# chngdickson/ov2slam

Measured on AMD Instinct MI355X. Metric: tracked_frames_per_sec, higher is better.
Workload: dtype u8/s16 fixed-point + f32

## Files before the change

### ov2slam_amd/csrc/klt.hip

```cpp
#include <cstdlib>

#include "ov2_internal.h"
#include "ov2_wave.h"

using namespace ov2wave;

namespace {

struct klt_params {
    int win, nlevels, max_iter;
    int wave_prio;
    double eps2;
    float err_th;
    double fb_th;
    float min_eig_thr;
    int rule33;
};

#define W_BITS 14

__device__ __forceinline__ void lk_weights(float a, float b, int &w00, int &w01, int &w10, int &w11)
{
    w00 = (int)__builtin_rintf((1.f - a) * (1.f - b) * (float)(1 << W_BITS));
    w01 = (int)__builtin_rintf(a * (1.f - b) * (float)(1 << W_BITS));
// ... 38 lines not shown
    constexpr int GSEG = klt_lds<WIN>::GSEG, NS = (WIN + 1) * GSEG, NK = (NS + GL - 1) / GL;
#pragma unroll
    for (int k = 0; k < NK; ++k) {
        const int sg = sub + GL * k;
        if (sg < NS) {
            const int row = sg / GSEG, part = sg - row * GSEG;
            *reinterpret_cast<uint4 *>(lg + sg * 16) =
                ld_b128(reinterpret_cast<const unsigned char *>(src + (size_t)row * gstride) + part * 16);
        }
    }
}

struct lds_col {
    const unsigned *q;
    unsigned sh;
};
__device__ __forceinline__ lds_col lds_col_of(const unsigned char *row0 , int byte_off)
{
    lds_col c;
    c.q = reinterpret_cast<const unsigned *>(row0 + (byte_off & ~3));
    c.sh = (unsigned)byte_off & 3u;
    return c;
}
__device__ __forceinline__ unsigned lds_pair(const lds_col &c, int row)
{
    const unsigned *q = c.q + 4 * row;
    return __builtin_amdgcn_alignbyte(q[1], q[0], c.sh);
}

typedef short ov2_s16x2 __attribute__((ext_vector_type(2)));

__device__ __forceinline__ int dot2(unsigned a, unsigned b, int c)
{
    return __builtin_amdgcn_sdot2(__builtin_bit_cast(ov2_s16x2, a), __builtin_bit_cast(ov2_s16x2, b), c, false);
}
__device__ __forceinline__ int dot2k(unsigned a, unsigned b, int k)
{
    int r;
    asm("v_dot2_i32_i16 %0, %1, %2, %3" : "=v"(r) : "v"(a), "v"(b), "s"(k));
    return r;
}
__device__ __forceinline__ unsigned spread_u8x2(unsigned t) { return __builtin_amdgcn_perm(0u, t, 0x0c010c00u); }
__device__ __forceinline__ unsigned pack_lo16(unsigned a, unsigned b) { return __builtin_amdgcn_perm(b, a, 0x05040100u); }
__device__ __forceinline__ unsigned pack_hi16(unsigned a, unsigned b) { return __builtin_amdgcn_perm(b, a, 0x07060302u); }
__device__ __forceinline__ unsigned pk_sub16(unsigned a, unsigned b)
{
    return __builtin_bit_cast(unsigned, (ov2_s16x2)(__builtin_bit_cast(ov2_s16x2, a) - __builtin_bit_cast(ov2_s16x2, b)));
}

typedef unsigned short ov2_u16x2 __attribute__((ext_vector_type(2)));
__device__ __forceinline__ unsigned pk_add16(unsigned a, unsigned b)
{
    return __builtin_bit_cast(unsigned, (ov2_u16x2)(__builtin_bit_cast(ov2_u16x2, a) + __builtin_bit_cast(ov2_u16x2, b)));
}
__device__ __forceinline__ unsigned pk_mul16(unsigned a, unsigned k)
{
    return __builtin_bit_cast(unsigned, (ov2_u16x2)(__builtin_bit_cast(ov2_u16x2, a) * (ov2_u16x2)((unsigned short)k)));
}
__device__ __forceinline__ unsigned pk_mad16(unsigned a, unsigned k, unsigned c)
{
    return __builtin_bit_cast(unsigned, (ov2_u16x2)(__builtin_bit_cast(ov2_u16x2, a) * (ov2_u16x2)((unsigned short)k) + __builtin_bit_cast(ov2_u16x2, c)));
}

template <int SH>
__device__ __forceinline__ unsigned shr_pack_hi(unsigned keep, unsigned acc)
{
    asm("v_lshrrev_b32_sdwa %0, %2, %1 dst_sel:WORD_1 dst_unused:UNUSED_PRESERVE src0_sel:DWORD src1_sel:DWORD" : "+v"(keep) : "v"(acc), "n"(SH));
    return keep;
}
template <int SH>
__device__ __forceinline__ unsigned ashr_pack_hi(unsigned keep, int acc)
{
    asm("v_ashrrev_i32_sdwa %0, %2, %1 dst_sel:WORD_1 dst_unused:UNUSED_PRESERVE src0_sel:DWORD src1_sel:DWORD" : "+v"(keep) : "v"(acc), "n"(SH));
    return keep;
}

struct level_ptrs {
    const unsigned char *img;
    const int *grad;
    int istride, gstride, w, h, rows;
    const unsigned char *base;
    unsigned img_o, grad_o;
};

__device__ __forceinline__ level_ptrs level_of(const ov2_pyr_view &v, int l, int b)
{
    level_ptrs p;
    const ov2_level_desc &L = v.lv[l];
    p.img = v.base + L.img_off + L.img_bstride * b;
    p.grad = reinterpret_cast<const int *>(v.base + L.grad_off + L.grad_bstride * b);
    p.istride = L.istride; p.gstride = L.gstride; p.w = L.w; p.h = L.h; p.rows = L.rows;
    p.base = v.base; p.img_o = (unsigned)(L.img_off + L.img_bstride * b); p.grad_o = (unsigned)(L.grad_off + L.grad_bstride * b);
    return p;
}

template <int WIN, int GL>
__device__ __forceinline__ int lk_level(const level_ptrs &I, const level_ptrs &J, int pad, int level, int max_level,
                                        bool run, float kx, float ky, float &nx_io, float &ny_io, int &status,
                                        float &err, const klt_params &P, int sub, unsigned &passes,
                                        unsigned char *lwI, unsigned char *lwJ, unsigned char *lg)
{
    constexpr int GROW = klt_lds<WIN>::GSEG * 4;
    constexpr int OC = WIN < GL ? WIN : GL;
    constexpr int NE = (WIN - OC) * WIN;
    constexpr int NR = (NE + GL - 1) / GL;
    constexpr int NRP = (NR + 1) / 2;
    constexpr int NP = (WIN + 1) / 2;
    const float FLT_SCALE = 1.f / (float)(1 << 20);
    const float half = (float)(WIN - 1) * 0.5f;
    const float lscale = __builtin_ldexpf(1.f, -level);
    float px = kx * lscale, py = ky * lscale;
    float nx, ny;
    if (level == max_level) { nx = nx_io * lscale; ny = ny_io * lscale; }
    else { nx = nx_io * 2.f; ny = ny_io * 2.f; }
    if (run) { nx_io = nx; ny_io = ny; }

    px -= half; py -= half;
    const int ipx = (int)floorf(px), ipy = (int)floorf(py);
    if (run && (ipx < -WIN || ipx >= I.w || ipy < -WIN || ipy >= I.h)) {
        if (level == 0) { status = 0; err = 0.f; }
        run = false;
    }
    if (!__any(run)) return 0;
    if (run) passes += 1u;
    int w00, w01, w10, w11;
    lk_weights(px - (float)ipx, py - (float)ipy, w00, w01, w10, w11);

    const bool col = sub < OC;
    const int sc = col ? sub : 0;
    unsigned Iv2[NP], Ix2[NP], Iy2[NP];
    unsigned IvE[NRP > 0 ? NRP : 1], IxE[NRP > 0 ? NRP : 1], IyE[NRP > 0 ? NRP : 1];
    int eoff[NR > 0 ? NR : 1];
    int sA11 = 0, sA12 = 0, sA22 = 0;
    {
        const unsigned W01 = pack_lo16((unsigned)w00, (unsigned)w01), W23 = pack_lo16((unsigned)w10, (unsigned)w11);
        const int bx0 = run ? (OV2_LM + ipx) : OV2_LM, by = run ? (ipy + pad) : pad;
        {
            const float sx = nx - half, sy = ny - half;
            const int inx0 = (int)floorf(sx), iny0 = (int)floorf(sy);
            const bool in0 = run && !(inx0 < -WIN || inx0 >= J.w || iny0 < -WIN || iny0 >= J.h);
            __syncthreads();
            const int jx0 = OV2_LM + (in0 ? inx0 : 0);
            stage_u8<WIN, GL>(I.img + (size_t)by * I.istride + (bx0 & ~3), I.istride, lwI, sub);
            stage_grad<WIN, GL>(I.grad + (size_t)by * I.gstride + bx0, I.gstride, lg, sub);
            stage_u8<WIN, GL>(J.img + (size_t)((in0 ? iny0 : 0) + pad) * J.istride + (jx0 & ~3), J.istride, lwJ, sub);
            __syncthreads();
        }
        const lds_col ci = lds_col_of(lwI, (bx0 & 3) + sc);
        const int *gp = reinterpret_cast<const int *>(lg) + sc;
        unsigned T = spread_u8x2(lds_pair(ci, 0));
        unsigned GX, GY;
        {
            const unsigned g0 = (unsigned)gp[0], g1 = (unsigned)gp[1];
            GX = pack_lo16(g0, g1); GY = pack_hi16(g0, g1);
        }
        const bool on = run && col;
        unsigned piv = 0, pix = 0, piy = 0;
#pragma unroll
        for (int y = 0; y < WIN; ++y) {
            gp += GROW;
            const unsigned B = spread_u8x2(lds_pair(ci, y + 1));
            const unsigned h0 = (unsigned)gp[0], h1 = (unsigned)gp[1];
            const unsigned HX = pack_lo16(h0, h1), HY = pack_hi16(h0, h1);
            const unsigned iv = (unsigned)dot2(B, W23, dot2k(T, W01, 1 << (W_BITS - 5 - 1))) >> (W_BITS - 5);
            int ix = dot2(HX, W23, dot2k(GX, W01, 1 << (W_BITS - 1))) >> W_BITS;
            int iy = dot2(HY, W23, dot2k(GY, W01, 1 << (W_BITS - 1))) >> W_BITS;
            if (y & 1) {
                Iv2[y >> 1] = pack_lo16(piv, iv); Ix2[y >> 1] = pack_lo16(pix, (unsigned)ix); Iy2[y >> 1] = pack_lo16(piy, (unsigned)iy);
            } else if (y == WIN - 1) {
                Iv2[y >> 1] = iv; Ix2[y >> 1] = (unsigned)ix & 0xffffu; Iy2[y >> 1] = (unsigned)iy & 0xffffu;
            } else {
                piv = iv; pix = (unsigned)ix; piy = (unsigned)iy;
            }
            T = B; GX = HX; GY = HY;
        }
        {
            const unsigned onm = on ? 0xffffffffu : 0u;
#pragma unroll
            for (int q = 0; q < NP; ++q) {
                Ix2[q] &= onm; Iy2[q] &= onm;
                sA11 = dot2(Ix2[q], Ix2[q], sA11); sA12 = dot2(Ix2[q], Iy2[q], sA12); sA22 = dot2(Iy2[q], Iy2[q], sA22);
            }
        }
#pragma unroll
        for (int r = 0; r < NR; ++r) {
            const int e = sub + GL * r;
            const bool ev = e < NE;
            const int ec = ev ? e : 0;
            const int ecol = OC + ec / WIN, erow = ec - (ec / WIN) * WIN;
            eoff[r] = erow * 16 + ecol;
            const lds_col ce = lds_col_of(lwI + erow * 16, (bx0 & 3) + ecol);
            const int *gpe = reinterpret_cast<const int *>(lg) + erow * GROW + ecol;
            const unsigned T0 = spread_u8x2(lds_pair(ce, 0)), T1 = spread_u8x2(lds_pair(ce, 1));
            const unsigned g0 = (unsigned)gpe[0], g1 = (unsigned)gpe[1];
            const unsigned h0 = (unsigned)gpe[GROW], h1 = (unsigned)gpe[GROW + 1];
            const unsigned iv = (unsigned)dot2(T1, W23, dot2k(T0, W01, 1 << (W_BITS - 5 - 1))) >> (W_BITS - 5);
            int ix = dot2(pack_lo16(h0, h1), W23, dot2k(pack_lo16(g0, g1), W01, 1 << (W_BITS - 1))) >> W_BITS;
            int iy = dot2(pack_hi16(h0, h1), W23, dot2k(pack_hi16(g0, g1), W01, 1 << (W_BITS - 1))) >> W_BITS;
            if (!(run && ev)) { ix = 0; iy = 0; }
            sA11 += __mul24(ix, ix); sA12 += __mul24(ix, iy); sA22 += __mul24(iy, iy);
            if (r & 1) {
                IvE[r >> 1] = pack_lo16(piv, iv); IxE[r >> 1] = pack_lo16(pix, (unsigned)ix); IyE[r >> 1] = pack_lo16(piy, (unsigned)iy);
            } else if (r == NR - 1) {
                IvE[r >> 1] = iv; IxE[r >> 1] = (unsigned)ix & 0xffffu; IyE[r >> 1] = (unsigned)iy & 0xffffu;
            } else {
                piv = iv; pix = (unsigned)ix; piy = (unsigned)iy;
            }
        }
    }
    const float A11 = (float)(double)row_sum_i32<GL>(sA11) * FLT_SCALE;
    const float A12 = (float)(double)row_sum_i32<GL>(sA12) * FLT_SCALE;
    const float A22 = (float)(double)row_sum_i32<GL>(sA22) * FLT_SCALE;
    float D = A11 * A22 - A12 * A12;
    const float min_eig = __fdiv_rn(A22 + A11 - __fsqrt_rn((A11 - A22) * (A11 - A22) + 4.f * A12 * A12),
                                    (float)(2 * WIN * WIN));
    if (run) {
        err = min_eig;
        if (min_eig < P.min_eig_thr || D < 1.1920929e-07f ) {
            if (level == 0) status = 0;
            run = false;
        }
    }
    D = __fdiv_rn(1.f, D);

    nx -= half; ny -= half;
    float pdx = 0.f, pdy = 0.f;
    int iters = 0;
    for (int j = 0; j < P.max_iter; ++j) {
        if (!__any(run)) break;
        const int inx = (int)floorf(nx), iny = (int)floorf(ny);
        if (run && (inx < -WIN || inx >= J.w || iny < -WIN || iny >= J.h)) {
            if (level == 0) status = 0;
            run = false;
        }
        lk_weights(nx - (float)inx, ny - (float)iny, w00, w01, w10, w11);
        if (j > 0) {
            __syncthreads();
            stage_u8<WIN, GL>(J.img + (size_t)((run ? iny : 0) + pad) * J.istride + ((OV2_LM + (run ? inx : 0)) & ~3), J.istride, lwJ, sub);
            __syncthreads();
        }
        const int jo = (run ? inx : 0) & 3;
        const lds_col cj = lds_col_of(lwJ, jo + sc);
        const unsigned W01 = pack_lo16((unsigned)w00, (unsigned)w01), W23 = pack_lo16((unsigned)w10, (unsigned)w11);
        int pb1 = 0, pb2 = 0;
        unsigned T = spread_u8x2(lds_pair(cj, 0));
#pragma unroll
        for (int q = 0; q < NP; ++q) {
            unsigned B = spread_u8x2(lds_pair(cj, 2 * q + 1));
            const unsigned j0 = (unsigned)dot2(B, W23, dot2k(T, W01, 1 << (W_BITS - 5 - 1))) >> (W_BITS - 5);
            T = B;
            unsigned j1 = 0;
            if (2 * q + 1 < WIN) {
                B = spread_u8x2(lds_pair(cj, 2 * q + 2));
                j1 = (unsigned)dot2(B, W23, dot2k(T, W01, 1 << (W_BITS - 5 - 1))) >> (W_BITS - 5);
                T = B;
            }
            const unsigned d2 = pk_sub16(j0 | (j1 << 16), Iv2[q]);
            pb1 = dot2(d2, Ix2[q], pb1);
            pb2 = dot2(d2, Iy2[q], pb2);
        }
#pragma unroll
        for (int q = 0; q < NRP; ++q) {
            const lds_col pe = lds_col_of(lwJ + (eoff[2 * q] & ~15), jo + (eoff[2 * q] & 15));
            const unsigned j0 = (unsigned)dot2(spread_u8x2(lds_pair(pe, 1)), W23,
                                               dot2k(spread_u8x2(lds_pair(pe, 0)), W01, 1 << (W_BITS - 5 - 1))) >> (W_BITS - 5);
            unsigned j1 = 0;
            if (2 * q + 1 < NR) {
                const lds_col pf = lds_col_of(lwJ + (eoff[2 * q + 1] & ~15), jo + (eoff[2 * q + 1] & 15));
                j1 = (unsigned)dot2(spread_u8x2(lds_pair(pf, 1)), W23,
                                    dot2k(spread_u8x2(lds_pair(pf, 0)), W01, 1 << (W_BITS - 5 - 1))) >> (W_BITS - 5);
            }
            const unsigned d2 = pk_sub16(j0 | (j1 << 16), IvE[q]);
            pb1 = dot2(d2, IxE[q], pb1);
            pb2 = dot2(d2, IyE[q], pb2);
        }
        float b1, b2;
        if (__all((unsigned)(pb1 + (1 << 27)) < (1u << 28) && (unsigned)(pb2 + (1 << 27)) < (1u << 28))) {
            b1 = (float)row_sum_i32<GL>(pb1) * FLT_SCALE;
            b2 = (float)row_sum_i32<GL>(pb2) * FLT_SCALE;
        } else {
            b1 = (float)row_sum_f64<GL>((double)pb1) * FLT_SCALE;
            b2 = (float)row_sum_f64<GL>((double)pb2) * FLT_SCALE;
        }
        const float dx = (A12 * b2 - A22 * b1) * D;
        const float dy = (A12 * b1 - A11 * b2) * D;
        if (run) {
            ++iters;
            nx += dx; ny += dy;
            nx_io = nx + half; ny_io = ny + half;
            if ((double)dx * dx + (double)dy * dy <= P.eps2) run = false;
            else if (j > 0 && fabsf(dx + pdx) <= 0.01f && fabsf(dy + pdy) <= 0.01f) {
                nx_io -= dx * 0.5f; ny_io -= dy * 0.5f;
                run = false;
            }
            pdx = dx; pdy = dy;
        }
    }
    return iters;
}

#ifndef KLT3_RROWS
#define KLT3_RROWS 14
#endif
#ifndef KLT3_RBYTES
#define KLT3_RBYTES 48
#endif
struct klt3 {
    static constexpr int RROWS = KLT3_RROWS, RBYTES = KLT3_RBYTES;
    static constexpr int RSZ = RROWS * RBYTES + 16;
    static constexpr int NLD = RBYTES == 48 ? RROWS : (2 * RROWS + 2) / 3;
    static constexpr int ROW_SPAN = RROWS - 10, ROW_MARGIN = ROW_SPAN / 2;
    static constexpr int COL_ALIGN = RBYTES == 48 ? 16 : 4;
    static constexpr int COL_LEAD = RBYTES == 48 ? 12 : 9, COL_SPAN = RBYTES == 48 ? 38 : 20;
};

template <int GL>
struct klt_map {
    static constexpr int KPW = 64 / GL;
    static __device__ __forceinline__ int slot(int tid) { return tid / GL; }
    static __device__ __forceinline__ int sub(int tid) { return tid & (GL - 1); }
    static __device__ __forceinline__ bool lane_ok(int) { return true; }
};
template <>
struct klt_map<3> {
    static constexpr int KPW = 21;
    static __device__ __forceinline__ int slot(int tid) { return min((tid * 171) >> 9, KPW - 1); }
    static __device__ __forceinline__ int sub(int tid) { return tid == 63 ? 0 : tid - 3 * ((tid * 171) >> 9); }
    static __device__ __forceinline__ bool lane_ok(int tid) { return tid != 63; }
};

template <int WIN, int GL>
struct klt_smem {
    static constexpr int BYTES = (64 / GL) * (2 * klt_lds<WIN>::WB + klt_lds<WIN>::GB);
};
template <int WIN>
struct klt_smem<WIN, 3> {
    static constexpr int BYTES = klt_map<3>::KPW * klt3::RSZ;
};

__device__ __forceinline__ int sum3_i32(int v, int c)
{
    const int t1 = v + dpp_i32<0x138>(v);
    const int t = v + dpp_i32<0x138>(t1);
    const int u1 = dpp_mov_i32<0x130>(t), u2 = dpp_mov_i32<0x130>(u1);
    return c == 2 ? t : (c == 1 ? u1 : u2);
}
__device__ __forceinline__ double sum3_f64(double v, int c)
{
    const double s1 = dpp_f64<0x138>(v), s2 = dpp_f64<0x138>(s1);
    const double t = (v + s1) + s2;
    const double u1 = dpp_f64<0x130>(t), u2 = dpp_f64<0x130>(u1);
    return c == 2 ? t : (c == 1 ? u1 : u2);
}

__device__ __forceinline__ unsigned klt3_pair_sel(unsigned k) { return 0x0c010c00u + k * 0x00010001u; }

__device__ __forceinline__ void klt3_region_origin(const level_ptrs &J, int pad, int inx, int iny, int &rr0, int &cc0)
{
    rr0 = min(max(iny + pad - klt3::ROW_MARGIN, 0), J.rows - klt3::RROWS);
    cc0 = min(max((OV2_LM + inx - klt3::COL_LEAD) & ~(klt3::COL_ALIGN - 1), 0), J.istride - klt3::RBYTES);
}

struct klt3_segs { uint4 v[klt3::NLD]; };
__device__ __forceinline__ void klt3_load_region(const level_ptrs &J, int rr0, int cc0, int c, klt3_segs &S)
{
    const unsigned o = J.img_o + (unsigned)(rr0 * J.istride + cc0);
#pragma unroll
    for (int t = 0; t < klt3::NLD; ++t) {
        unsigned a;
        if (klt3::RBYTES == 48) a = o + (unsigned)(t * J.istride + 16 * c);
        else {
            const int sg = min(3 * t + c, 2 * klt3::RROWS - 1);
            a = o + (unsigned)((sg >> 1) * J.istride + (sg & 1) * 16);
        }
        S.v[t] = ld_b128(J.base + (size_t)a);
    }
}
__device__ __forceinline__ void klt3_store_region(const klt3_segs &S, int c, bool store, unsigned char *lj)
{
    if (store) {
#pragma unroll
        for (int t = 0; t < klt3::NLD; ++t) {
            if (klt3::RBYTES == 48) *reinterpret_cast<uint4 *>(lj + t * klt3::RBYTES + 16 * c) = S.v[t];
            else if (3 * t + c < 2 * klt3::RROWS) *reinterpret_cast<uint4 *>(lj + (3 * t + c) * 16) = S.v[t];
        }
    }
}

template <int WIN>
__device__ __forceinline__ int lk_level3(const level_ptrs &I, const level_ptrs &J, int pad, int level, int max_level,
                                         bool run, float kx, float ky, float &nx_io, float &ny_io, int &status,
                                         float &err, const klt_params &P, int c, bool lane_ok, unsigned &passes,
                                         unsigned char *lj)
{
    static_assert(WIN == 9, "three lanes x three columns");
    constexpr int NPX = 3 * WIN, NQ = (NPX + 1) / 2;
    const float FLT_SCALE = 1.f / (float)(1 << 20);
    const float half = (float)(WIN - 1) * 0.5f;
    const float lscale = __builtin_ldexpf(1.f, -level);
    float px = kx * lscale, py = ky * lscale;
    float nx, ny;
    if (level == max_level) { nx = nx_io * lscale; ny = ny_io * lscale; }
    else { nx = nx_io * 2.f; ny = ny_io * 2.f; }
    if (run) { nx_io = nx; ny_io = ny; }

    px -= half; py -= half;
    const int ipx = (int)floorf(px), ipy = (int)floorf(py);
    if (run && (ipx < -WIN || ipx >= I.w || ipy < -WIN || ipy >= I.h)) {
        if (level == 0) { status = 0; err = 0.f; }
        run = false;
    }
    if (!__any(run)) return 0;
    if (run) passes += 1u;
    int w00, w01, w10, w11;
    lk_weights(px - (float)ipx, py - (float)ipy, w00, w01, w10, w11);

    unsigned Iv2[NQ], Ix2[NQ], Iy2[NQ];
    int sA11 = 0, sA12 = 0, sA22 = 0;
    int rr0, cc0;
    {
        const float sx = nx - half, sy = ny - half;
        const int inx0 = (int)floorf(sx), iny0 = (int)floorf(sy);
        const bool in0 = run && !(inx0 < -WIN || inx0 >= J.w || iny0 < -WIN || iny0 >= J.h);
        klt3_region_origin(J, pad, in0 ? inx0 : 0, in0 ? iny0 : 0, rr0, cc0);
        const int bx0 = (run ? (OV2_LM + ipx) : OV2_LM) + 3 * c, by = run ? (ipy + pad) : pad;
        const int ax = bx0 - 1;
        const unsigned io = I.img_o + (unsigned)(by * I.istride + (ax & ~3));
        const unsigned shI = (unsigned)ax & 3u;
        struct row3 { unsigned x, y, z; };
        row3 irow[WIN + 3];
#define KLT3_LOAD_ROW(p)                                                                                                  \
    do {                                                                                                                  \
        const int dr = (p) == 0 ? (by > 0 ? -1 : 0) : ((p) == WIN + 2 ? (by + WIN + 1 < I.rows ? WIN + 1 : WIN) : (p) - 1); \
        __builtin_memcpy(&irow[p], __builtin_assume_aligned(I.base + (size_t)(io + (unsigned)(dr * I.istride)), 4), 12);   \
    } while (0)
        constexpr int R1 = 6;
        __syncthreads();
        klt3_segs S;
        klt3_load_region(J, rr0, cc0, c, S);
#pragma unroll
        for (int p = 0; p < R1; ++p) KLT3_LOAD_ROW(p);
        klt3_store_region(S, c, lane_ok, lj);
        __syncthreads();
#pragma unroll
        for (int p = R1; p < WIN + 3; ++p) KLT3_LOAD_ROW(p);
#undef KLT3_LOAD_ROW

        const unsigned W01 = pack_lo16((unsigned)w00, (unsigned)w01), W23 = pack_lo16((unsigned)w10, (unsigned)w11);
        const int x0 = ipx + 3 * c;
        const unsigned wlim = (run && lane_ok) ? (unsigned)I.w : 0u, hlim = (run && lane_ok) ? (unsigned)I.h : 0u;
        unsigned cm[2];
#pragma unroll
        for (int j = 0; j < 2; ++j)
            cm[j] = ((unsigned)(x0 + 2 * j) < wlim ? 0xffffu : 0u) | ((unsigned)(x0 + 2 * j + 1) < wlim ? 0xffff0000u : 0u);
        const unsigned cmi[3] = {cm[0], __builtin_amdgcn_perm(cm[1], cm[0], 0x05040302u), cm[1]};
        unsigned W01g[3], W23g[3];
#pragma unroll
        for (int i = 0; i < 3; ++i) { W01g[i] = W01 & cmi[i]; W23g[i] = W23 & cmi[i]; }
        unsigned selI[4];
#pragma unroll
        for (int k = 0; k < 4; ++k) selI[k] = klt3_pair_sel(shI + (unsigned)k);
        unsigned Pm[2][3] = {};
        unsigned Hd[3][2] = {}, Sm[3][2] = {};
        unsigned GXp[3] = {0, 0, 0}, GYp[3] = {0, 0, 0};
        unsigned piv = 0, pix = 0, piy = 0;
#pragma unroll
        for (int p = 0; p < WIN + 3; ++p) {
            unsigned P[5];
#pragma unroll
            for (int k = 0; k < 4; ++k) P[k] = __builtin_amdgcn_perm(irow[p].y, irow[p].x, selI[k]);
            P[4] = __builtin_amdgcn_perm(irow[p].z, irow[p].y, selI[0]);
#pragma unroll
            for (int j = 0; j < 2; ++j) {
                Hd[0][j] = Hd[1][j]; Hd[1][j] = Hd[2][j]; Sm[0][j] = Sm[1][j]; Sm[1][j] = Sm[2][j];
                Hd[2][j] = pk_sub16(P[2 * j + 2], P[2 * j]);
                Sm[2][j] = pk_mad16(P[2 * j + 1], 10u, pk_mul16(pk_add16(P[2 * j], P[2 * j + 2]), 3u));
            }
            if (p >= 2) {
                const unsigned rm = (unsigned)(ipy + p - 2) < hlim ? 0xffffffffu : 0u;
                unsigned GX[3], GY[3];
#pragma unroll
                for (int j = 0; j < 2; ++j) {
                    GX[2 * j] = pk_mad16(Hd[1][j], 10u, pk_mul16(pk_add16(Hd[0][j], Hd[2][j]), 3u)) & rm;
                    GY[2 * j] = pk_sub16(Sm[2][j], Sm[0][j]) & rm;
                }
                GX[1] = __builtin_amdgcn_perm(GX[2], GX[0], 0x05040302u); GY[1] = __builtin_amdgcn_perm(GY[2], GY[0], 0x05040302u);
                if (p >= 3) {
                    const int y = p - 3;
#pragma unroll
                    for (int i = 0; i < 3; ++i) {
                        const int e = 3 * y + i;
                        const unsigned av = (unsigned)dot2(Pm[1][i], W23, dot2k(Pm[0][i], W01, 1 << (W_BITS - 5 - 1)));
                        const int ax_ = dot2(GX[i], W23g[i], dot2k(GXp[i], W01g[i], 1 << (W_BITS - 1)));
                        const int ay_ = dot2(GY[i], W23g[i], dot2k(GYp[i], W01g[i], 1 << (W_BITS - 1)));
                        if (e & 1) {
                            Iv2[e >> 1] = shr_pack_hi<W_BITS - 5>(piv, av);
                            Ix2[e >> 1] = ashr_pack_hi<W_BITS>(pix, ax_);
                            Iy2[e >> 1] = ashr_pack_hi<W_BITS>(piy, ay_);
                        } else if (e == NPX - 1) {
                            Iv2[e >> 1] = av >> (W_BITS - 5);
                            Ix2[e >> 1] = (unsigned)(ax_ >> W_BITS) & 0xffffu; Iy2[e >> 1] = (unsigned)(ay_ >> W_BITS) & 0xffffu;
                        } else {
                            piv = av >> (W_BITS - 5); pix = (unsigned)(ax_ >> W_BITS); piy = (unsigned)(ay_ >> W_BITS);
                        }
                    }
                }
#pragma unroll
                for (int j = 0; j < 3; ++j) { GXp[j] = GX[j]; GYp[j] = GY[j]; }
            }
#pragma unroll
            for (int j = 0; j < 3; ++j) { Pm[0][j] = Pm[1][j]; Pm[1][j] = P[j + 1]; }
        }
#pragma unroll
        for (int q = 0; q < NQ; ++q) {
            sA11 = dot2(Ix2[q], Ix2[q], sA11); sA12 = dot2(Ix2[q], Iy2[q], sA12); sA22 = dot2(Iy2[q], Iy2[q], sA22);
        }
    }
    const float A11 = (float)(double)sum3_i32(sA11, c) * FLT_SCALE;
    const float A12 = (float)(double)sum3_i32(sA12, c) * FLT_SCALE;
    const float A22 = (float)(double)sum3_i32(sA22, c) * FLT_SCALE;
    float D = A11 * A22 - A12 * A12;
    const float min_eig = __fdiv_rn(A22 + A11 - __fsqrt_rn((A11 - A22) * (A11 - A22) + 4.f * A12 * A12),
                                    (float)(2 * WIN * WIN));
    if (run) {
        err = min_eig;
        if (min_eig < P.min_eig_thr || D < 1.1920929e-07f ) {
            if (level == 0) status = 0;
            run = false;
        }
    }
    D = __fdiv_rn(1.f, D);

    nx -= half; ny -= half;
    float pdx = 0.f, pdy = 0.f;
    int iters = 0;
    for (int j = 0; j < P.max_iter; ++j) {
        if (!__any(run)) break;
        const int inx = (int)floorf(nx), iny = (int)floorf(ny);
        if (run && (inx < -WIN || inx >= J.w || iny < -WIN || iny >= J.h)) {
            if (level == 0) status = 0;
            run = false;
        }
        int w00j, w01j, w10j, w11j;
        lk_weights(nx - (float)inx, ny - (float)iny, w00j, w01j, w10j, w11j);
        int rb = run ? iny + pad - rr0 : 0, cb = run ? OV2_LM + inx - cc0 : 0;
        const bool out = (unsigned)rb > (unsigned)klt3::ROW_SPAN || (unsigned)cb > (unsigned)klt3::COL_SPAN;
        if (__any(out)) {
            __syncthreads();
            if (out) {
                klt3_region_origin(J, pad, inx, iny, rr0, cc0);
                klt3_segs S;
                klt3_load_region(J, rr0, cc0, c, S);
                klt3_store_region(S, c, lane_ok, lj);
                rb = iny + pad - rr0; cb = OV2_LM + inx - cc0;
            }
            __syncthreads();
        }
        const unsigned W01 = pack_lo16((unsigned)w00j, (unsigned)w01j), W23 = pack_lo16((unsigned)w10j, (unsigned)w11j);
        const int cq = cb + 3 * c;
        const unsigned *q = reinterpret_cast<const unsigned *>(lj + rb * klt3::RBYTES + (cq & ~3));
        unsigned selJ[3];
#pragma unroll
        for (int i = 0; i < 3; ++i) selJ[i] = klt3_pair_sel(((unsigned)cq & 3u) + (unsigned)i);
        int pb1 = 0, pb2 = 0;
        unsigned T[3];
#pragma unroll
        for (int i = 0; i < 3; ++i) T[i] = __builtin_amdgcn_perm(q[1], q[0], selJ[i]);
        unsigned pj = 0;
#pragma unroll
        for (int y = 0; y < WIN; ++y) {
            const unsigned *qr = q + (klt3::RBYTES / 4) * (y + 1);
            unsigned B[3];
#pragma unroll
            for (int i = 0; i < 3; ++i) B[i] = __builtin_amdgcn_perm(qr[1], qr[0], selJ[i]);
#pragma unroll
            for (int i = 0; i < 3; ++i) {
                const int e = 3 * y + i;
                const unsigned aj = (unsigned)dot2(B[i], W23, dot2k(T[i], W01, 1 << (W_BITS - 5 - 1)));
                if ((e & 1) || e == NPX - 1) {
                    const unsigned d2 = pk_sub16((e & 1) ? shr_pack_hi<W_BITS - 5>(pj, aj) : (aj >> (W_BITS - 5)), Iv2[e >> 1]);
                    pb1 = dot2(d2, Ix2[e >> 1], pb1);
                    pb2 = dot2(d2, Iy2[e >> 1], pb2);
                } else {
                    pj = aj >> (W_BITS - 5);
                }
                T[i] = B[i];
            }
        }
        float b1, b2;
        if (__all((unsigned)(pb1 + (1 << 27)) < (1u << 28) && (unsigned)(pb2 + (1 << 27)) < (1u << 28))) {
            b1 = (float)sum3_i32(pb1, c) * FLT_SCALE;
            b2 = (float)sum3_i32(pb2, c) * FLT_SCALE;
        } else {
            b1 = (float)sum3_f64((double)pb1, c) * FLT_SCALE;
            b2 = (float)sum3_f64((double)pb2, c) * FLT_SCALE;
        }
        const float dx = (A12 * b2 - A22 * b1) * D;
        const float dy = (A12 * b1 - A11 * b2) * D;
        if (run) {
            ++iters;
            nx += dx; ny += dy;
            nx_io = nx + half; ny_io = ny + half;
            if ((double)dx * dx + (double)dy * dy <= P.eps2) run = false;
            else if (j > 0 && fabsf(dx + pdx) <= 0.01f && fabsf(dy + pdy) <= 0.01f) {
                nx_io -= dx * 0.5f; ny_io -= dy * 0.5f;
                run = false;
            }
            pdx = dx; pdy = dy;
        }
    }
    return iters;
}

template <int WIN, int GL>
__device__ __forceinline__ int lk_pass(const level_ptrs &I, const level_ptrs &J, int pad, int level, int max_level, bool run,
                                       float kx, float ky, float &nx_io, float &ny_io, int &status, float &err,
                                       const klt_params &P, int sub, bool lane_ok, unsigned &passes, unsigned char *smem, int slot)
{
    if constexpr (GL == 3) {
        return lk_level3<WIN>(I, J, pad, level, max_level, run, kx, ky, nx_io, ny_io, status, err, P, sub, lane_ok, passes,
                              smem + slot * klt3::RSZ);
    } else {
        constexpr int KPW = 64 / GL, WB = klt_lds<WIN>::WB, GB = klt_lds<WIN>::GB;
        return lk_level<WIN, GL>(I, J, pad, level, max_level, run, kx, ky, nx_io, ny_io, status, err, P, sub, passes,
                                 smem + slot * WB, smem + KPW * WB + slot * WB, smem + 2 * KPW * WB + slot * GB);
    }
}

struct __attribute__((aligned(16))) klt_handover { float fx, fy, err; unsigned work; };

template <int WIN, int GL>
__device__ __forceinline__ int fb_track(const ov2_pyr_view &pv, const ov2_pyr_view &cv, int b, bool act, float kx,
                                          float ky, float &fx, float &fy, const klt_params &P, int nlevels, int sub,
                                          bool lane_ok, unsigned &work, unsigned char *smem, int slot,
                                          int l_hi, int l_lo, float err0, unsigned work0, float &err_out)
{
    int status = 1;
    float err = err0;
    unsigned it = work0 & 0xffffu, passes = work0 >> 16;
    for (int l = l_hi; l >= l_lo; --l) {
        const level_ptrs I = level_of(pv, l, b), J = level_of(cv, l, b);
        it += lk_pass<WIN, GL>(I, J, pv.pad, l, nlevels, act, kx, ky, fx, fy, status, err, P, sub, lane_ok, passes, smem, slot);
    }
    if (l_lo > 0) {
        work = it | (passes << 16);
        err_out = err;
        return 0;
    }
    const int W0 = cv.lv[0].w, H0 = cv.lv[0].h;
    int ok = act && status && !(err > P.err_th) &&
             (1.f <= fx && fx < (float)W0 - 1.f && 1.f <= fy && fy < (float)H0 - 1.f);
    int st2 = 1;
    float e2 = 0.f, bx = kx, by = ky;
    {
        const level_ptrs I = level_of(cv, 0, b), J = level_of(pv, 0, b);
        it += lk_pass<WIN, GL>(I, J, cv.pad, 0, 0, ok != 0, fx, fy, bx, by, st2, e2, P, sub, lane_ok, passes, smem, slot);
    }
    if (ok) {
        if (!st2) ok = 0;
        else {
            const float dx = kx - bx, dy = ky - by;
            const double nrm = __dsqrt_rn((double)dx * dx + (double)dy * dy);
            if (nrm > P.fb_th) ok = 0;
        }
    }
    work = it | (passes << 16);
    return ok;
}

template <int WIN, int GL>
__device__ __forceinline__ int fb_track(const ov2_pyr_view &pv, const ov2_pyr_view &cv, int b, bool act, float kx,
                                          float ky, float &fx, float &fy, const klt_params &P, int nlevels, int sub,
                                          bool lane_ok, unsigned &work, unsigned char *smem, int slot)
{
    float err;
    return fb_track<WIN, GL>(pv, cv, b, act, kx, ky, fx, fy, P, nlevels, sub, lane_ok, work, smem, slot, nlevels, 0, 0.f, 0u, err);
}

#define KLT_GL8_MIN_KPS 65536
#ifndef KLT_STEREO_SPLIT_DEFAULT
#define KLT_STEREO_SPLIT_DEFAULT 0
#endif
#ifndef KLT_SPLIT_C_FIRST
#define KLT_SPLIT_C_FIRST 1
#endif
#ifndef KLT_WAVE_CAP
#define KLT_WAVE_CAP 4
#endif
#ifndef KLT3_WAVE_MIN
#define KLT3_WAVE_MIN 2
#endif
#define KLT_WAVES(W, G) ((G) == 3 ? KLT3_WAVE_MIN : 1), KLT_WAVE_CAP

template <int WIN, int KLT_GL>
__global__ __launch_bounds__(64) __attribute__((amdgpu_waves_per_eu(KLT_WAVES(WIN, KLT_GL)))) void klt_fb_kernel(ov2_pyr_view pv, ov2_pyr_view cv, klt_params P, int n,
                                                    const float2 *__restrict__ kps, float2 *__restrict__ priors,
                                                    unsigned char *__restrict__ status,
                                                    const int *__restrict__ img_idx, unsigned *__restrict__ iters)
{
    __shared__ __attribute__((aligned(16))) unsigned char smem[klt_smem<WIN, KLT_GL>::BYTES];
    ov2wave::set_wave_prio(P.wave_prio);
    using M = klt_map<KLT_GL>;
    constexpr int KLT_KPW = M::KPW;
    const int slot = M::slot((int)threadIdx.x), sub = M::sub((int)threadIdx.x), i = blockIdx.x * KLT_KPW + slot;
    const bool lane_ok = M::lane_ok((int)threadIdx.x);
    const bool act = i < n && lane_ok;
    const int ii = i < n ? i : 0;
    const int b = img_idx ? img_idx[ii] : 0;
    const float2 kp = kps[ii];
    float2 pr = priors[ii];
    unsigned work = 0;
    const int ok = fb_track<WIN, KLT_GL>(pv, cv, b, act, kp.x, kp.y, pr.x, pr.y, P, P.nlevels, sub, lane_ok, work, smem, slot);
    if (act && sub == 0) {
        priors[i] = pr;
        status[i] = (unsigned char)ok;
        if (iters) iters[i] = work;
    }
}


#define KLT_COMPACT_KPT 8
#define KLT_COMPACT_KPWG (256 * KLT_COMPACT_KPT)
__global__ __launch_bounds__(256) void klt_compact_kernel(int n, const unsigned char *__restrict__ has_prior,
                                                          unsigned *__restrict__ iters, int *__restrict__ list_a,
                                                          int *__restrict__ list_b, unsigned *__restrict__ cnt,
                                                          int *__restrict__ p3p_req, int batch, int wave_prio)
{
    ov2wave::set_wave_prio(wave_prio);
    __shared__ int wsum[2][4];
    __shared__ int wbase[2];
    const int lane = threadIdx.x & 63, wv = threadIdx.x >> 6;
    const int f0 = blockIdx.x * KLT_COMPACT_KPWG + wv * (64 * KLT_COMPACT_KPT) + lane;
    unsigned char hp[KLT_COMPACT_KPT];
#pragma unroll
    for (int k = 0; k < KLT_COMPACT_KPT; ++k) hp[k] = f0 + 64 * k < n ? has_prior[f0 + 64 * k] : 0;
    int pos[KLT_COMPACT_KPT];
    int ta = 0, tb = 0;
#pragma unroll
    for (int k = 0; k < KLT_COMPACT_KPT; ++k) {
        const bool v = f0 + 64 * k < n, p = hp[k] != 0;
        const unsigned long long ba = __ballot(v && p), bb = __ballot(v && !p);
        const int ra = ta + (int)__builtin_amdgcn_mbcnt_hi((unsigned)(ba >> 32), __builtin_amdgcn_mbcnt_lo((unsigned)ba, 0u));
        const int rb = tb + (int)__builtin_amdgcn_mbcnt_hi((unsigned)(bb >> 32), __builtin_amdgcn_mbcnt_lo((unsigned)bb, 0u));
        ta += __popcll(ba); tb += __popcll(bb);
        pos[k] = p ? ra : rb;
    }
    if (lane == 0) { wsum[0][wv] = ta; wsum[1][wv] = tb; }
    __syncthreads();
    if (threadIdx.x < 2) {
        const int q = threadIdx.x;
        const int tot = wsum[q][0] + wsum[q][1] + wsum[q][2] + wsum[q][3];
        wbase[q] = tot ? (int)atomicAdd(&cnt[q], (unsigned)tot) : 0;
    }
    __syncthreads();
    int oa = wbase[0], ob = wbase[1];
    for (int k = 0; k < wv; ++k) { oa += wsum[0][k]; ob += wsum[1][k]; }
#pragma unroll
    for (int k = 0; k < KLT_COMPACT_KPT; ++k) {
        const int f = f0 + 64 * k;
        if (f < n) {
            const bool p = hp[k] != 0;
            (p ? list_a : list_b)[(p ? oa : ob) + pos[k]] = f;
            if (iters) iters[p ? n + f : f] = 0;
        }
    }
    if (p3p_req)
        for (int k = blockIdx.x * 256 + threadIdx.x; k < batch; k += gridDim.x * 256) p3p_req[k] = 0;
}

__device__ __forceinline__ void klt_stage1_finish(bool mine, bool is_a, int i, int b, int n, int ok, float2 pr, unsigned work,
                                                  float2 *__restrict__ out_xy, unsigned char *__restrict__ out_status,
                                                  unsigned *__restrict__ counts, unsigned *__restrict__ iters,
                                                  unsigned *__restrict__ cnt, int *__restrict__ list_c)
{
    if (mine) {
        out_xy[i] = pr;
        out_status[i] = (unsigned char)ok;
        if (iters) iters[is_a ? i : n + i] = work;
        if (is_a) atomicAdd(&counts[64 * b + (i & 63)], 1u + ((unsigned)ok << 16));
    }
    const bool retry = mine && is_a && !ok;
    const unsigned long long rm = __ballot(retry);
    if (rm) {
        const int lane = (int)threadIdx.x, leader = __ffsll((long long)rm) - 1;
        int base = 0;
        if (lane == leader) base = (int)atomicAdd(&cnt[2], (unsigned)__popcll(rm));
        base = __shfl(base, leader);
        if (retry) list_c[base + __popcll(rm & ((1ull << lane) - 1ull))] = i;
    }
}

template <int WIN, int KLT_GL, bool SPLIT>
__global__ __launch_bounds__(64) __attribute__((amdgpu_waves_per_eu(KLT_WAVES(WIN, KLT_GL)))) void klt_stage1_kernel(ov2_pyr_view pv, ov2_pyr_view cv, klt_params P, int n,
                                                        const float2 *__restrict__ kps,
                                                        const float2 *__restrict__ prior,
                                                        const int *__restrict__ img_idx, float2 *__restrict__ out_xy,
                                                        unsigned char *__restrict__ out_status,
                                                        unsigned *__restrict__ counts ,
                                                        unsigned *__restrict__ iters, const int *__restrict__ list_a,
                                                        const int *__restrict__ list_b, unsigned *__restrict__ cnt,
                                                        int *__restrict__ list_c,
                                                        int b_word ,
                                                        int split_k ,
                                                        klt_handover *__restrict__ hand )
{
    __shared__ __attribute__((aligned(16))) unsigned char smem[klt_smem<WIN, KLT_GL>::BYTES];
    using M = klt_map<KLT_GL>;
    constexpr int KLT_KPW = M::KPW;
    const int total_a = (int)cnt[0], total_b = (int)cnt[b_word];
    const int groups_b = (total_b + KLT_KPW - 1) / KLT_KPW;
    const bool is_a = (int)blockIdx.x >= groups_b;
    const int g = is_a ? (int)blockIdx.x - groups_b : (int)blockIdx.x;
    const int total = is_a ? total_a : total_b;
    if (g * KLT_KPW >= total) return;
    ov2wave::set_wave_prio(P.wave_prio);
    const int slot = M::slot((int)threadIdx.x), sub = M::sub((int)threadIdx.x), idx = g * KLT_KPW + slot;
    const bool lane_ok = M::lane_ok((int)threadIdx.x);
    const bool act = idx < total && lane_ok;
    const int i = (is_a ? list_a : list_b)[idx < total ? idx : total - 1];
    const float2 kp = kps[i];
    const int b = img_idx ? img_idx[i] : 0;
    float2 pr = (is_a || !P.rule33) ? prior[i] : kp;
    unsigned work = 0;
    const int nl = is_a ? min(1, pv.nlevels - 1) : P.nlevels;
    const bool upper = SPLIT && !is_a;
    float err;
    const int ok = fb_track<WIN, KLT_GL>(pv, cv, b, act, kp.x, kp.y, pr.x, pr.y, P, nl, sub, lane_ok, work, smem, slot, nl,
                                         upper ? split_k + 1 : 0, 0.f, 0u, err);
    if (upper) {
        if (act && sub == 0) hand[i] = klt_handover{pr.x, pr.y, err, work};
        return;
    }
    klt_stage1_finish(act && sub == 0, is_a, i, b, n, ok, pr, work, out_xy, out_status, counts, iters, cnt, list_c);
}

template <int WIN, int KLT_GL>
__global__ __launch_bounds__(64) __attribute__((amdgpu_waves_per_eu(KLT_WAVES(WIN, KLT_GL)))) void klt_stage2_kernel(ov2_pyr_view pv, ov2_pyr_view cv, klt_params P, int n,
                                                        const float2 *__restrict__ kps,
                                                        const int *__restrict__ img_idx, float2 *__restrict__ out_xy,
                                                        unsigned char *__restrict__ out_status,
                                                        const unsigned *__restrict__ counts, int *__restrict__ p3p_req,
                                                        unsigned *__restrict__ iters, const int *__restrict__ list_c,
                                                        const unsigned *__restrict__ cnt, int batch,
                                                        unsigned *__restrict__ next_counts, int next_words,
                                                        const int *__restrict__ list_b, int b_word,
                                                        const float2 *__restrict__ prior,
                                                        int split_k ,
                                                        const klt_handover *__restrict__ hand)
{
    __shared__ __attribute__((aligned(16))) unsigned char smem[klt_smem<WIN, KLT_GL>::BYTES];
    using M = klt_map<KLT_GL>;
    constexpr int KLT_KPW = M::KPW;
    const int slot = M::slot((int)threadIdx.x), sub = M::sub((int)threadIdx.x);
    const bool lane_ok = M::lane_ok((int)threadIdx.x);
    for (int q = blockIdx.x * 64 + threadIdx.x; q < next_words; q += gridDim.x * 64) next_counts[q] = 0u;
    auto tally = [&](int b, int &n3, int &good) {
        n3 = 0; good = 0;
        if constexpr (KLT_GL == 3) {
            for (int q = sub; q < 64; q += 3) {
                const unsigned cw = counts[64 * b + q];
                n3 += (int)(cw & 0xffffu); good += (int)(cw >> 16);
            }
            n3 = sum3_i32(n3, sub); good = sum3_i32(good, sub);
        } else {
            for (int q = 0; q < 64 / KLT_GL; ++q) {
                const unsigned cw = counts[64 * b + sub * (64 / KLT_GL) + q];
                n3 += (int)(cw & 0xffffu); good += (int)(cw >> 16);
            }
            n3 = row_sum_i32<KLT_GL>(n3); good = row_sum_i32<KLT_GL>(good);
        }
    };
    if (p3p_req && P.rule33) {
        for (int b0 = blockIdx.x * KLT_KPW; b0 < batch; b0 += gridDim.x * KLT_KPW) {
            const int b = b0 + slot;
            int n3, good;
            tally(min(b, batch - 1), n3, good);
            if (b < batch && lane_ok && sub == 0 && n3 > 0 && (double)good < 0.33 * (double)n3) p3p_req[b] = 1;
        }
    }
    const int total_b = (int)cnt[b_word], total_c = (int)cnt[2];
    const bool b_first = split_k < 0 || !KLT_SPLIT_C_FIRST;
    const int groups_1 = ((b_first ? total_b : total_c) + KLT_KPW - 1) / KLT_KPW;
    const bool first = (int)blockIdx.x < groups_1;
    const bool is_b = first == b_first;
    const int g = first ? (int)blockIdx.x : (int)blockIdx.x - groups_1;
    const int total = is_b ? total_b : total_c;
    if (g * KLT_KPW >= total) return;
    ov2wave::set_wave_prio(P.wave_prio);
    const int idx = g * KLT_KPW + slot;
    const bool act = idx < total && lane_ok;
    const int i = (is_b ? list_b : list_c)[idx < total ? idx : total - 1];
    const int b = img_idx ? img_idx[i] : 0;
    const float2 kp = kps[i];
    float2 pr;
    int l_hi = P.nlevels;
    float err0 = 0.f;
    unsigned work0 = 0;
    if (is_b) {
        if (split_k >= 0) {
            const klt_handover hr = hand[i];
            pr = make_float2(hr.fx, hr.fy);
            err0 = hr.err; work0 = hr.work; l_hi = split_k;
        } else {
            pr = prior[i];
        }
    } else {
        int n3, good;
        tally(b, n3, good);
        const bool drop = P.rule33 && n3 > 0 && (double)good < 0.33 * (double)n3;
        pr = drop ? kp : out_xy[i];
    }
    unsigned work = 0;
    float err;
    const int ok = fb_track<WIN, KLT_GL>(pv, cv, b, act, kp.x, kp.y, pr.x, pr.y, P, P.nlevels, sub, lane_ok, work, smem, slot,
                                         l_hi, 0, err0, work0, err);
    if (act && sub == 0) {
        out_xy[i] = pr;
        out_status[i] = (unsigned char)ok;
        if (iters) iters[n + i] = work;
    }
}

int klt_lanes_for(const ov2_ctx *c, int n, int win, const ov2_pyr *a, const ov2_pyr *b)
{
    static const int env = [] { const char *e = getenv("OV2_KLT_LANES"); return e ? atoi(e) : 0; }();
    const int forced = c->klt_lanes ? c->klt_lanes : env;
    const bool fits32 = a->buf->bytes < (1ull << 32) && b->buf->bytes < (1ull << 32);
    if (forced == 8 || forced == 16 || (forced == 3 && win == 9 && fits32)) return forced;
    if (win == 9 && fits32) return 3;
    return n >= KLT_GL8_MIN_KPS ? 8 : 16;
}

ov2_status make_params(ov2_ctx *c, const ov2_pyr *prev, const ov2_pyr *cur, int win, int nlevels, int max_iter,
                       float eps, float err_th, float fb_th, klt_params *P)
{
    if (!prev || !cur) return ov2_set_err(c, OV2_ERR_INVALID, "null pyramid");
    const ov2_pyr_view &a = prev->buf->view, &b = cur->buf->view;
    if (a.nlevels != b.nlevels || a.pad != b.pad || a.batch != b.batch || a.lv[0].w != b.lv[0].w ||
        a.lv[0].h != b.lv[0].h)
        return ov2_set_err(c, OV2_ERR_INVALID, "prev/cur pyramids differ in geometry");
    if (win < 3 || win > 11 || (win & 1) == 0 || win > a.pad)
        return ov2_set_err(c, OV2_ERR_INVALID, "win=%d unsupported (odd, 3..11, <= pyramid pad %d)", win, a.pad);
    if (nlevels < 0) return ov2_set_err(c, OV2_ERR_INVALID, "nlevels < 0");
    if (a.nlevels < nlevels + 1) nlevels = a.nlevels - 1;
    P->win = win;
    P->wave_prio = c->wave_prio;
    P->nlevels = nlevels;
    P->max_iter = max_iter < 0 ? 0 : (max_iter > 100 ? 100 : max_iter);
    double e = (double)eps;
    if (e < 0.) e = 0.;
    if (e > 10.) e = 10.;
    P->eps2 = e * e;
    P->err_th = err_th;
    P->fb_th = (double)fb_th;
    P->min_eig_thr = 1e-4f;
    P->rule33 = 1;
    return OV2_OK;
}

}

extern "C" ov2_status ov2_klt_set_lanes(ov2_ctx *c, int lanes)
{
    if (!c) return OV2_ERR_INVALID;
    if (lanes != 0 && lanes != 3 && lanes != 8 && lanes != 16) return ov2_set_err(c, OV2_ERR_INVALID, "lanes per keypoint: 0 (auto), 3, 8 or 16");
    c->klt_lanes = lanes;
    return OV2_OK;
}

extern "C" ov2_status ov2_klt_set_stereo_split(ov2_ctx *c, int k)
{
    if (!c) return OV2_ERR_INVALID;
    c->klt_stereo_split = k < 0 ? -1 : k;
    return OV2_OK;
}

extern "C" ov2_status ov2_klt_track_fb_dev(ov2_ctx *c, const ov2_pyr *prev, const ov2_pyr *cur, int win, int nlevels,
                                           int max_iter, float eps, float err_th, float fb_th, int n,
                                           const float *d_kps, float *d_priors, uint8_t *d_status,
                                           const int32_t *d_img_idx, uint32_t *d_iters)
{
    if (!c) return OV2_ERR_INVALID;
    if (n == 0) return OV2_OK;
    if (n < 0 || !d_kps || !d_priors || !d_status) return ov2_set_err(c, OV2_ERR_INVALID, "null/negative argument");
    klt_params P;
    ov2_status s = make_params(c, prev, cur, win, nlevels, max_iter, eps, err_th, fb_th, &P);
    if (s != OV2_OK) return s;
    OV2_HIP(c, hipSetDevice(c->device));
    if ((s = ov2_pyr_wait_ready(c, prev)) != OV2_OK || (s = ov2_pyr_wait_ready(c, cur)) != OV2_OK) return s;
    const int lanes = klt_lanes_for(c, n, win, prev, cur);
    if (lanes != 3 && ((s = ov2_pyr_need_grad(c, prev)) != OV2_OK || (s = ov2_pyr_need_grad(c, cur)) != OV2_OK)) return s;
#define KLT_FB_GL(W, G)                                                                                        \
    OV2_LAUNCH(c, OV2_K_KLT_FB, (klt_fb_kernel<W, G>), dim3((n + klt_map<G>::KPW - 1) / klt_map<G>::KPW), dim3(64), 0, c->stream,    \
               prev->buf->view, cur->buf->view, P, n, reinterpret_cast<const float2 *>(d_kps),                 \
               reinterpret_cast<float2 *>(d_priors), d_status, d_img_idx, d_iters)
// ... 151 lines not shown
```

Measured before the change: 294,000.

## Use 32-byte LDS region rows, batch region staging, and cap GL3 waves per EU

Fixes the GL=3 KLT path to a 32-byte-wide shared-memory search region with a new load addressing scheme, and splits region loading and storing into two batches separated by scheduling barriers so fewer VGPRs hold in-flight segments. It also caps waves per EU for the GL=3 kernel at 3 and uses an empty asm clobber of a high VGPR to push the allocator toward a fixed budget. The aim is lower register pressure and smaller region transfers. The narrower region may trigger more reloads when tracked points drift, and the occupancy cap limits latency hiding.

Measured after the change: 305,000, median of 6. +3.7%, better.

```diff
diff --git a/ov2slam_amd/csrc/klt.hip b/ov2slam_amd/csrc/klt.hip
--- a/ov2slam_amd/csrc/klt.hip
+++ b/ov2slam_amd/csrc/klt.hip
@@ -364,16 +364,21 @@
 #ifndef KLT3_RROWS
 #define KLT3_RROWS 14
 #endif
-#ifndef KLT3_RBYTES
-#define KLT3_RBYTES 48
+#ifndef KLT3_WAVES
+#define KLT3_WAVES 3
+#endif
+#if KLT3_WAVES == 3
+#define KLT3_VGPR_CLAIM "v135"
+#elif KLT3_WAVES == 2
+#define KLT3_VGPR_CLAIM "v175"
 #endif
 struct klt3 {
-    static constexpr int RROWS = KLT3_RROWS, RBYTES = KLT3_RBYTES;
+    static constexpr int RROWS = KLT3_RROWS, RBYTES = 32;
     static constexpr int RSZ = RROWS * RBYTES + 16;
-    static constexpr int NLD = RBYTES == 48 ? RROWS : (2 * RROWS + 2) / 3;
+    static constexpr int NLD = (2 * RROWS + 2) / 3;
     static constexpr int ROW_SPAN = RROWS - 10, ROW_MARGIN = ROW_SPAN / 2;
-    static constexpr int COL_ALIGN = RBYTES == 48 ? 16 : 4;
-    static constexpr int COL_LEAD = RBYTES == 48 ? 12 : 9, COL_SPAN = RBYTES == 48 ? 38 : 20;
+    static constexpr int COL_ALIGN = 4;
+    static constexpr int COL_LEAD = 9, COL_SPAN = 20;
 };
 
 template <int GL>
@@ -423,29 +428,44 @@
     cc0 = min(max((OV2_LM + inx - klt3::COL_LEAD) & ~(klt3::COL_ALIGN - 1), 0), J.istride - klt3::RBYTES);
 }
 
-struct klt3_segs { uint4 v[klt3::NLD]; };
-__device__ __forceinline__ void klt3_load_region(const level_ptrs &J, int rr0, int cc0, int c, klt3_segs &S)
+#ifndef KLT3_REGION_BATCHES
+#define KLT3_REGION_BATCHES 2
+#endif
+template <int T0, int T1>
+struct klt3_segs { uint4 v[T1 - T0]; };
+template <int T0, int T1>
+__device__ __forceinline__ void klt3_load_region(const level_ptrs &J, int rr0, int cc0, int c, klt3_segs<T0, T1> &S)
 {
     const unsigned o = J.img_o + (unsigned)(rr0 * J.istride + cc0);
-#pragma unroll
-    for (int t = 0; t < klt3::NLD; ++t) {
-        unsigned a;
-        if (klt3::RBYTES == 48) a = o + (unsigned)(t * J.istride + 16 * c);
-        else {
-            const int sg = min(3 * t + c, 2 * klt3::RROWS - 1);
-            a = o + (unsigned)((sg >> 1) * J.istride + (sg & 1) * 16);
-        }
-        S.v[t] = ld_b128(J.base + (size_t)a);
-    }
-}
-__device__ __forceinline__ void klt3_store_region(const klt3_segs &S, int c, bool store, unsigned char *lj)
+    const unsigned a0 = o + (unsigned)((c >> 1) * J.istride + (c & 1) * 16);
+    const unsigned a1 = a0 + (unsigned)((c & 1) ? 2 * J.istride - 16 : J.istride + 16);
+#pragma unroll
+    for (int t = T0; t < T1; ++t) {
+        unsigned a = ((t & 1) ? a1 : a0) + (unsigned)((t >> 1) * 3 * J.istride);
+        if (3 * t + 2 >= 2 * klt3::RROWS && 3 * t + c >= 2 * klt3::RROWS) a = ((t & 1) ? a0 : a1) + (unsigned)(((t - 1) >> 1) * 3 * J.istride);
+        S.v[t - T0] = ld_b128(J.base + (size_t)a);
+    }
+}
+template <int T0, int T1>
+__device__ __forceinline__ void klt3_store_region(const klt3_segs<T0, T1> &S, int c, bool store, unsigned char *lj)
 {
     if (store) {
 #pragma unroll
-        for (int t = 0; t < klt3::NLD; ++t) {
-            if (klt3::RBYTES == 48) *reinterpret_cast<uint4 *>(lj + t * klt3::RBYTES + 16 * c) = S.v[t];
-            else if (3 * t + c < 2 * klt3::RROWS) *reinterpret_cast<uint4 *>(lj + (3 * t + c) * 16) = S.v[t];
-        }
+        for (int t = T0; t < T1; ++t) {
+            if (3 * t + 2 < 2 * klt3::RROWS || 3 * t + c < 2 * klt3::RROWS) *reinterpret_cast<uint4 *>(lj + (3 * t + c) * 16) = S.v[t - T0];
+        }
+    }
+}
+template <int B, int NB>
+__device__ __forceinline__ void klt3_stage_region(const level_ptrs &J, int rr0, int cc0, int c, bool store, unsigned char *lj)
+{
+    if constexpr (B < NB) {
+        constexpr int T0 = klt3::NLD * B / NB, T1 = klt3::NLD * (B + 1) / NB;
+        klt3_segs<T0, T1> S;
+        klt3_load_region(J, rr0, cc0, c, S);
+        klt3_store_region(S, c, store, lj);
+        __builtin_amdgcn_sched_barrier(0);
+        klt3_stage_region<B + 1, NB>(J, rr0, cc0, c, store, lj);
     }
 }
 
@@ -456,6 +476,9 @@
                                          unsigned char *lj)
 {
     static_assert(WIN == 9, "three lanes x three columns");
+#ifdef KLT3_VGPR_CLAIM
+    asm volatile("" ::: KLT3_VGPR_CLAIM);
+#endif
     constexpr int NPX = 3 * WIN, NQ = (NPX + 1) / 2;
     const float FLT_SCALE = 1.f / (float)(1 << 20);
     const float half = (float)(WIN - 1) * 0.5f;
@@ -498,11 +521,16 @@
     } while (0)
         constexpr int R1 = 6;
         __syncthreads();
-        klt3_segs S;
-        klt3_load_region(J, rr0, cc0, c, S);
-#pragma unroll
-        for (int p = 0; p < R1; ++p) KLT3_LOAD_ROW(p);
-        klt3_store_region(S, c, lane_ok, lj);
+        {
+            constexpr int T1 = klt3::NLD / KLT3_REGION_BATCHES;
+            klt3_segs<0, T1> S;
+            klt3_load_region(J, rr0, cc0, c, S);
+#pragma unroll
+            for (int p = 0; p < R1; ++p) KLT3_LOAD_ROW(p);
+            klt3_store_region(S, c, lane_ok, lj);
+        }
+        __builtin_amdgcn_sched_barrier(0);
+        klt3_stage_region<1, KLT3_REGION_BATCHES>(J, rr0, cc0, c, lane_ok, lj);
         __syncthreads();
 #pragma unroll
         for (int p = R1; p < WIN + 3; ++p) KLT3_LOAD_ROW(p);
@@ -611,9 +639,7 @@
             __syncthreads();
             if (out) {
                 klt3_region_origin(J, pad, inx, iny, rr0, cc0);
-                klt3_segs S;
-                klt3_load_region(J, rr0, cc0, c, S);
-                klt3_store_region(S, c, lane_ok, lj);
+                klt3_stage_region<0, KLT3_REGION_BATCHES>(J, rr0, cc0, c, lane_ok, lj);
                 rb = iny + pad - rr0; cb = OV2_LM + inx - cc0;
             }
             __syncthreads();
@@ -752,7 +778,7 @@
 #ifndef KLT3_WAVE_MIN
 #define KLT3_WAVE_MIN 2
 #endif
-#define KLT_WAVES(W, G) ((G) == 3 ? KLT3_WAVE_MIN : 1), KLT_WAVE_CAP
+#define KLT_WAVES(W, G) ((G) == 3 ? KLT3_WAVE_MIN : 1), ((G) == 3 ? KLT3_WAVES : KLT_WAVE_CAP)
 
 template <int WIN, int KLT_GL>
 __global__ __launch_bounds__(64) __attribute__((amdgpu_waves_per_eu(KLT_WAVES(WIN, KLT_GL)))) void klt_fb_kernel(ov2_pyr_view pv, ov2_pyr_view cv, klt_params P, int n,
```
